# genomematt/xenomapper

Hardware: AMD Instinct MI355X
Metric: read-pairs/sec classified (higher is better)
Workload: dtype int32; 1 GPU; configs[1]: 50000000 PE 2x150 pairs/GPU, AS/XS, liberal, HBM-resident; pairs_per_gpu=50000000, step=xm_classify_compact_dev: classify+count, scan, scatter (3 launches)

## Files before the change

xenomapper_amd/csrc/xm_kernels.hip:

```cpp
#include <hip/hip_runtime.h>
#include <stdint.h>
#include <stdlib.h>

#include "xm_kernels.h"

namespace xm {

template <typename T>
__device__ __forceinline__ uint32_t mapping_state(T a1, T x1, T a2, T x2, T m)
{
    const bool low1 = a1 <= m;
    const bool low2 = a2 <= m;
    const bool prim = (a1 > m) && (low2 || a1 > a2);
    const bool sec  = (a2 > m) && (low1 || a2 > a1);
    const bool spec1 = (x1 == T(0)) || (a1 > x1);
    const bool spec2 = (x2 == T(0)) || (a2 > x2);
    uint32_t s = 6u;
    s = sec ? (spec2 ? 1u : 3u) : s;
    s = (a1 == a2) ? 4u : s;
    s = prim ? (spec1 ? 0u : 2u) : s;
    s = (low1 && low2) ? 5u : s;
    return s;
}

template <>
__device__ __forceinline__ uint32_t mapping_state<int32_t>(int32_t a1, int32_t x1, int32_t a2, int32_t x2, int32_t m)
{
    const bool low1 = a1 <= m, low2 = a2 <= m;
    const bool gt = a1 > a2, lt = a2 > a1;
    const bool spec1 = (x1 == 0) || (a1 > x1);
    const bool spec2 = (x2 == 0) || (a2 > x2);
    uint32_t s = spec2 ? 1u : 3u;
    s = (gt || lt) ? s : 4u;
    s = (!low1 && (low2 || gt)) ? (spec1 ? 0u : 2u) : s;
    s = (low1 && low2) ? 5u : s;
    return s;
}

__device__ __forceinline__ uint32_t bin_of_code(int mode, uint32_t c)
{
    const uint32_t f = (c >> 3) & 7u, r = c & 7u;
    const uint32_t lo = f < r ? f : r;
    const uint32_t hi = f < r ? r : f;
    uint32_t b;
    if (mode == XM_MODE_SE) {
        b = r > 6u ? 6u : r;
    } else if (mode == XM_MODE_PE_LIBERAL) {
        b = lo;
    } else {
        b = (hi == 5u) ? 5u
          : ((hi == 4u) || (((f ^ r) & 1u) != 0u)) ? 4u
          : lo;
    }
    if (mode != XM_MODE_SE) b = (hi > 5u) ? 6u : b;
    return (c == XM_NO_UNIT) ? 7u : b;
}

template <typename T> struct Vec4;
typedef int32_t v4i32 __attribute__((ext_vector_type(4)));
typedef int32_t v4i32_a4 __attribute__((ext_vector_type(4), aligned(4)));
typedef uint32_t v8u32_a4 __attribute__((ext_vector_type(8), aligned(4)));
typedef double  v4f64 __attribute__((ext_vector_type(4)));
template <> struct Vec4<int32_t> { typedef v4i32 type; };
template <> struct Vec4<double>  { typedef v4f64 type; };

template <typename T> __device__ __forceinline__ T absent_value();
template <> __device__ __forceinline__ int32_t absent_value<int32_t>() { return INT32_MIN; }
template <> __device__ __forceinline__ double  absent_value<double>()  { return -__builtin_huge_val(); }

template <typename T, bool NT, bool FULL = false>
__device__ __forceinline__ void load4(const T *__restrict__ col, uint64_t r0, uint64_t n, T out[4])
{
    typedef typename Vec4<T>::type V;
    if (FULL || r0 + 4 <= n) {
        const V *p = reinterpret_cast<const V *>(col + r0);
        const V v = NT ? __builtin_nontemporal_load(p) : *p;
        out[0] = v.x; out[1] = v.y; out[2] = v.z; out[3] = v.w;
    } else {
#pragma unroll
        for (int j = 0; j < 4; ++j) out[j] = (r0 + j < n) ? col[r0 + j] : absent_value<T>();
    }
}

template <typename T, bool NT>
__device__ __forceinline__ void load4_wg(const T *__restrict__ wg, uint32_t byte_off, T out[4])
{
    typedef typename Vec4<T>::type V;
    const V *p = reinterpret_cast<const V *>(reinterpret_cast<const char *>(wg) + byte_off);
    const V v = NT ? __builtin_nontemporal_load(p) : *p;
    out[0] = v.x; out[1] = v.y; out[2] = v.z; out[3] = v.w;
}

__device__ __forceinline__ uint32_t wave_scan_incl(uint32_t v)
{
    v += (uint32_t)__builtin_amdgcn_update_dpp(0, (int)v, 0x111, 0xf, 0xf, false);
    v += (uint32_t)__builtin_amdgcn_update_dpp(0, (int)v, 0x112, 0xf, 0xf, false);
    v += (uint32_t)__builtin_amdgcn_update_dpp(0, (int)v, 0x114, 0xf, 0xf, false);
    v += (uint32_t)__builtin_amdgcn_update_dpp(0, (int)v, 0x118, 0xf, 0xf, false);
    v += (uint32_t)__builtin_amdgcn_update_dpp(0, (int)v, 0x142, 0xa, 0xf, false);
    v += (uint32_t)__builtin_amdgcn_update_dpp(0, (int)v, 0x143, 0xc, 0xf, false);
    return v;
}

__device__ __forceinline__ uint32_t lane_value(uint32_t v, int lane)
{
    return (uint32_t)__builtin_amdgcn_readlane((int)v, lane);
}

#ifdef XM_LOCKSTEP_HOST
__device__ __forceinline__ void lds_settle(int line = __builtin_LINE()) { ls::settle(line); }
#else
__device__ __forceinline__ void lds_settle()
{
    asm volatile("s_waitcnt lgkmcnt(0)" ::: "memory");
}
#endif

#ifdef XM_LOCKSTEP_HOST
#define XM_LAUNCH(kernel, grid, block, st, ...) do { (void)(st); ls::launch(grid, block, [&] { kernel(__VA_ARGS__); }); } while (0)
#else
#define XM_LAUNCH(kernel, grid, block, st, ...) kernel<<<grid, block, 0, st>>>(__VA_ARGS__)
#endif

#if defined(XM_LOCKSTEP_HOST) && defined(LS_SUBSETS)
#define XM_IF_LANES(cond) if (ls::Subset xm_lanes_{static_cast<bool>(cond), __builtin_LINE()}; xm_lanes_.taken)
#else
#define XM_IF_LANES(cond) if (cond)
#endif

#define XM_HREP 8
#define XM_COUNT_LDS_WORDS (64 * XM_HREP + 16)

struct CountSink {
    uint32_t *gran_counts;
    uint32_t *part_tot;
    unsigned long long *counts_rep;
    uint8_t *bins4;
    uint32_t gran_stride;
    int mode;
    uint32_t blk0;
};

__device__ __forceinline__ void count_flush(uint32_t *lds, uint32_t granule, const CountSink &sink)
{
    const uint32_t lane = threadIdx.x & 63u;
    uint32_t *misc = lds + 64 * XM_HREP;
    const uint4 h0 = *reinterpret_cast<const uint4 *>(lds + lane * XM_HREP);
    const uint4 h1 = *reinterpret_cast<const uint4 *>(lds + lane * XM_HREP + 4);
    const uint32_t s = h0.x + h0.y + h0.z + h0.w + h1.x + h1.y + h1.z + h1.w;
    if (s != 0u) {
        atomicAdd(&sink.counts_rep[(granule % XM_COUNT_REPLICAS) * 64u + lane], (unsigned long long)s);
        atomicAdd(&misc[8u + bin_of_code(sink.mode, lane)], s);
    }
    lds_settle();
    if (lane < 8u) {
        const uint32_t v = misc[8u + lane];
        sink.gran_counts[(uint64_t)lane * sink.gran_stride + granule] = v;
        if (v != 0u) atomicAdd(&sink.part_tot[((granule & (XM_PART_REPLICAS - 1u)) * 8u + lane) * XM_PART_STRIDE + granule / XM_PART_GRAN], v);
    }
}

template <int BLOCK>
__device__ __forceinline__ void count_units(const uint32_t c[4], uint32_t *lds, const CountSink &sink)
{
    const uint32_t lane = threadIdx.x & 63u;
    const uint32_t rep = lane & (XM_HREP - 1u);
#pragma unroll
    for (int j = 0; j < 4; ++j) {
        const bool unit = c[j] != XM_NO_UNIT;
        if (__ballot(unit) == 0ull) continue;
        if (unit) atomicAdd(&lds[(c[j] & 63u) * XM_HREP + rep], 1u);
    }
    lds_settle();
    uint32_t arrived = 0;
    if (lane == 0u) arrived = atomicAdd(&lds[64 * XM_HREP], 1u);
    arrived = (uint32_t)__builtin_amdgcn_readfirstlane((int)arrived);
    if (arrived != (uint32_t)(BLOCK / 64 - 1)) return;
    lds_settle();
    count_flush(lds, blockIdx.x + sink.blk0, sink);
}

template <int MODE, bool HAS6>
__device__ __forceinline__ uint32_t unit_bin(uint32_t c)
{
    if (MODE == XM_MODE_SE) return c == XM_NO_UNIT ? 7u : (c & 7u);
    const uint32_t f = (c >> 3) & 7u, r = c & 7u;
    const uint32_t lo = f < r ? f : r, hi = f < r ? r : f;
    uint32_t b = lo;
    if (MODE == XM_MODE_PE_CONSERVATIVE) {
        b = (((f ^ r) & 1u) != 0u || hi == 4u) ? 4u : b;
        b = (hi == 5u) ? 5u : b;
    }
    if (HAS6) b = (hi > 5u) ? 6u : b;
    return c == XM_NO_UNIT ? 7u : b;
}

template <int MODE, bool HAS6>
__device__ __forceinline__ uint32_t unit_bin_of(uint32_t f, uint32_t r, bool unit)
{
    uint32_t b;
    if (MODE == XM_MODE_SE) {
        b = r;
    } else {
        const uint32_t lo = f < r ? f : r, hi = f < r ? r : f;
        b = lo;
        if (MODE == XM_MODE_PE_CONSERVATIVE) {
            b = (((f ^ r) & 1u) != 0u || hi == 4u) ? 4u : b;
            b = (hi == 5u) ? 5u : b;
        }
        if (HAS6) b = (hi > 5u) ? 6u : b;
    }
    return unit ? b : 7u;
}

template <typename T, bool PAIRED, int BLOCK, bool FULL, bool COUNTS, int BINMODE>
__device__ __forceinline__ void classify_finish(const T a1[4], const T x1[4], const T a2[4], const T x2[4], T m,
                                                uint32_t mb, uint32_t halo, uint32_t *last_state,
                                                uint8_t *__restrict__ code, uint64_t r0, uint64_t n,
                                                uint32_t *count_lds, const CountSink &sink)
{
    const uint32_t lane = threadIdx.x & 63u;
    const uint32_t wave = threadIdx.x >> 6;
    uint32_t s[4];
#pragma unroll
    for (int j = 0; j < 4; ++j) s[j] = mapping_state<T>(a1[j], x1[j], a2[j], x2[j], m);

    uint32_t c[4], fwd[4] = {0, 0, 0, 0};
    if (PAIRED) {
        uint32_t prev = (uint32_t)__builtin_amdgcn_update_dpp(0, (int)s[3], 0x138, 0xf, 0xf, false);
        if (lane == 63) last_state[wave] = s[3];
        __syncthreads();
        if (lane == 0) prev = (wave == 0) ? halo : last_state[wave - 1];
        c[0] = (mb & 1u) ? ((prev << 3) | s[0]) : XM_NO_UNIT;
        c[1] = (mb & 2u) ? ((s[0] << 3) | s[1]) : XM_NO_UNIT;
        c[2] = (mb & 4u) ? ((s[1] << 3) | s[2]) : XM_NO_UNIT;
        c[3] = (mb & 8u) ? ((s[2] << 3) | s[3]) : XM_NO_UNIT;
        fwd[0] = prev; fwd[1] = s[0]; fwd[2] = s[1]; fwd[3] = s[2];
    } else {
        if (COUNTS) __syncthreads();
#pragma unroll
        for (int j = 0; j < 4; ++j) c[j] = ((mb >> j) & 1u) ? s[j] : XM_NO_UNIT;
    }

    if (FULL || r0 + 4 <= n) {
        if (code != nullptr) *reinterpret_cast<uint32_t *>(code + r0) = c[0] | (c[1] << 8) | (c[2] << 16) | (c[3] << 24);
    } else {
#pragma unroll
        for (int j = 0; j < 4; ++j)
            if (code != nullptr && r0 + j < n) code[r0 + j] = (uint8_t)c[j];
    }
    if (BINMODE >= 0) {
        uint32_t nib = 0;
#pragma unroll
        for (int j = 0; j < 4; ++j) nib |= unit_bin_of<BINMODE, sizeof(T) == 8>(fwd[j], s[j], ((mb >> j) & 1u) != 0u) << (4 * j);
        reinterpret_cast<uint16_t *>(sink.bins4)[r0 >> 2] = (uint16_t)nib;
    }
    if (COUNTS) count_units<BLOCK>(c, count_lds, sink);
}

template <typename T, bool PAIRED, bool NT, int BLOCK, bool FULL>
__device__ __forceinline__ void classify_load(const T *__restrict__ as1, const T *__restrict__ xs1,
                                              const T *__restrict__ as2, const T *__restrict__ xs2,
                                              const uint8_t *__restrict__ unit_bits8, T m, uint64_t n, uint64_t wg,
                                              T a1[4], T x1[4], T a2[4], T x2[4], uint32_t &mb, uint32_t &halo)
{
    const uint64_t g = wg * BLOCK + threadIdx.x;
    const uint64_t r0 = g * 4;
    mb = 0;
    halo = 0;
    if (FULL) {
        const uint32_t wave = (uint32_t)__builtin_amdgcn_readfirstlane((int)(threadIdx.x >> 6));
        const uint32_t lane = threadIdx.x & 63u;
        const v8u32_a4 mw = *reinterpret_cast<const v8u32_a4 *>(unit_bits8 + wg * (BLOCK / 2) + wave * 32u);
        load4<T, NT, true>(as1, r0, n, a1);
        load4<T, NT, true>(xs1, r0, n, x1);
        load4<T, NT, true>(as2, r0, n, a2);
        load4<T, NT, true>(xs2, r0, n, x2);
        uint32_t d = mw[0];
#pragma unroll
        for (uint32_t k = 1; k < 8u; ++k) d = ((lane >> 3) == k) ? mw[k] : d;
        mb = (d >> ((lane & 7u) * 4u)) & 0xFu;
        if (PAIRED && wave == 0u) {
            if (wg == 0) {
                if (lane == 0u) mb &= ~1u;
            } else if (mw[0] & 1u) {
                const uint64_t h = wg * (BLOCK * 4) - 1;
                halo = mapping_state<T>(as1[h], xs1[h], as2[h], xs2[h], m);
            }
        }
    } else {
        if (r0 < n) mb = (uint32_t)(unit_bits8[g >> 1] >> ((g & 1u) * 4u)) & 0xFu;
        load4<T, NT, false>(as1, r0, n, a1);
        load4<T, NT, false>(xs1, r0, n, x1);
        load4<T, NT, false>(as2, r0, n, a2);
        load4<T, NT, false>(xs2, r0, n, x2);
        if (r0 + 4 > n) mb &= (r0 < n) ? ((1u << (uint32_t)(n - r0)) - 1u) : 0u;
        if (PAIRED && threadIdx.x == 0) {
            if (r0 == 0) {
                mb &= ~1u;
            } else if (mb & 1u) {
                const uint64_t h = r0 - 1;
                halo = mapping_state<T>(as1[h], xs1[h], as2[h], xs2[h], m);
            }
        }
    }
}

template <typename T, bool PAIRED, bool NT, int BLOCK, bool FULL, bool COUNTS, int BINMODE>
__device__ __forceinline__ void classify_body(const T *__restrict__ as1, const T *__restrict__ xs1,
                                              const T *__restrict__ as2, const T *__restrict__ xs2,
                                              const uint8_t *__restrict__ unit_bits8, T m,
                                              uint8_t *__restrict__ code, uint64_t n, uint32_t *last_state,
                                              uint32_t *count_lds, const CountSink &sink)
{
    const uint64_t wg = (uint64_t)blockIdx.x + sink.blk0;
    const uint64_t r0 = (wg * BLOCK + threadIdx.x) * 4;
    T a1[4], x1[4], a2[4], x2[4];
    uint32_t mb, halo;
    classify_load<T, PAIRED, NT, BLOCK, FULL>(as1, xs1, as2, xs2, unit_bits8, m, n, wg, a1, x1, a2, x2, mb, halo);
    classify_finish<T, PAIRED, BLOCK, FULL, COUNTS, BINMODE>(a1, x1, a2, x2, m, mb, halo, last_state, code, r0, n, count_lds, sink);
}

template <int BLOCK>
__device__ __forceinline__ void count_lds_clear(uint32_t *count_lds)
{
    for (uint32_t k = threadIdx.x; k < (uint32_t)XM_COUNT_LDS_WORDS; k += BLOCK) count_lds[k] = 0;
}

template <typename T, bool PAIRED, bool NT, int BLOCK, bool COUNTS, int BINMODE>
__global__ void __launch_bounds__(BLOCK)
classify_kernel(const T *__restrict__ as1, const T *__restrict__ xs1,
                const T *__restrict__ as2, const T *__restrict__ xs2,
                const uint8_t *__restrict__ unit_bits8, T m,
                uint8_t *__restrict__ code, uint64_t n, CountSink sink)
{
    __shared__ uint32_t last_state[BLOCK / 64];
    __shared__ __attribute__((aligned(16))) uint32_t count_lds[COUNTS ? XM_COUNT_LDS_WORDS : 4];
    if (COUNTS) count_lds_clear<BLOCK>(count_lds);
    if (((uint64_t)blockIdx.x + sink.blk0 + 1) * (BLOCK * 4) <= n)
        classify_body<T, PAIRED, NT, BLOCK, true, COUNTS, BINMODE>(as1, xs1, as2, xs2, unit_bits8, m, code, n, last_state, count_lds, sink);
    else
        classify_body<T, PAIRED, NT, BLOCK, false, COUNTS, BINMODE>(as1, xs1, as2, xs2, unit_bits8, m, code, n, last_state, count_lds, sink);
}


__device__ __attribute__((noinline)) uint4 load_codes16_tail(const uint8_t *__restrict__ code, uint64_t base, uint64_t n)
{
    uint32_t w[4];
    for (int k = 0; k < 4; ++k) {
        uint32_t acc = 0;
        for (int j = 0; j < 4; ++j) {
            const uint64_t i = base + 4 * k + j;
            const uint32_t c = (i < n) ? (uint32_t)code[i] : XM_NO_UNIT;
            acc |= c << (8 * j);
        }
        w[k] = acc;
    }
    return make_uint4(w[0], w[1], w[2], w[3]);
}

__device__ __forceinline__ void load_codes16(const uint8_t *__restrict__ code, uint64_t base, uint64_t n,
                                             uint32_t w[4])
{
    uint4 v;
    if (base + 16 <= n) v = *reinterpret_cast<const uint4 *>(code + base);
    else v = load_codes16_tail(code, base, n);
    w[0] = v.x; w[1] = v.y; w[2] = v.z; w[3] = v.w;
}

__device__ __attribute__((noinline)) uint32_t load_codes4_tail(const uint8_t *__restrict__ code, uint64_t base, uint64_t n)
{
    uint32_t acc = 0;
    for (int j = 0; j < 4; ++j) {
        const uint64_t i = base + j;
        const uint32_t c = (i < n) ? (uint32_t)code[i] : XM_NO_UNIT;
        acc |= c << (8 * j);
    }
    return acc;
}

__global__ void __launch_bounds__(XM_BLOCK)
hist_kernel(const uint8_t *__restrict__ code, uint64_t n, uint32_t n_gran, CountSink sink)
{
    __shared__ __attribute__((aligned(16))) uint32_t lds_all[XM_BLOCK / 64][XM_COUNT_LDS_WORDS];
    const uint32_t lane = threadIdx.x & 63u, wave = threadIdx.x >> 6;
    uint32_t *lds = lds_all[wave];
    const uint32_t g = blockIdx.x * (XM_BLOCK / 64) + wave;
    if (g >= n_gran) return;
    for (uint32_t k = lane; k < (uint32_t)XM_COUNT_LDS_WORDS; k += 64u) lds[k] = 0;

    constexpr int TILES = XM_GRAN / 1024;
    const uint64_t rec0 = (uint64_t)g * XM_GRAN;
    uint32_t w[TILES][4];
#pragma unroll
    for (int k = 0; k < TILES; ++k) load_codes16(code, rec0 + (uint64_t)k * 1024u + lane * 16u, n, w[k]);
    lds_settle();

    const uint32_t rep = lane & (XM_HREP - 1u);
    uint32_t common = w[0][0] & 0xFFu;
    if (common == XM_NO_UNIT) common = (w[0][0] >> 8) & 0xFFu;
    common = (uint32_t)__builtin_amdgcn_readfirstlane((int)common);
    uint32_t n_common = 0;
#pragma unroll
    for (int k = 0; k < TILES; ++k) {
#pragma unroll
        for (int j = 0; j < 16; ++j) {
            const uint32_t c = (w[k][j >> 2] >> (8 * (j & 3))) & 0xFFu;
            const bool unit = c != XM_NO_UNIT;
            if (__ballot(unit) == 0ull) continue;
            const bool same = unit && c == common;
            n_common += same ? 1u : 0u;
            if (unit && !same) atomicAdd(&lds[(c & 63u) * XM_HREP + rep], 1u);
        }
    }
    if (n_common) atomicAdd(&lds[(common & 63u) * XM_HREP + rep], n_common);
    lds_settle();
    count_flush(lds, g, sink);
}

#define XM_SCAN_THREADS 1024
__device__ __forceinline__ unsigned long long block_sum_1024(unsigned long long v, unsigned long long *wsum)
{
    v += __shfl_xor(v, 1, 64);  v += __shfl_xor(v, 2, 64);  v += __shfl_xor(v, 4, 64);
    v += __shfl_xor(v, 8, 64);  v += __shfl_xor(v, 16, 64); v += __shfl_xor(v, 32, 64);
    if ((threadIdx.x & 63u) == 0u) wsum[threadIdx.x >> 6] = v;
    __syncthreads();
    unsigned long long total = 0;
#pragma unroll
    for (int w = 0; w < XM_SCAN_THREADS / 64; ++w) total += wsum[w];
    return total;
}

__global__ void __launch_bounds__(XM_SCAN_THREADS)
scan_kernel(const uint32_t *__restrict__ gran_counts, uint32_t n_gran, uint32_t gran_stride,
            const uint32_t *__restrict__ part_tot, uint32_t *__restrict__ gran_off,
            unsigned long long *__restrict__ bin_totals,
            unsigned long long *__restrict__ counts_rep, unsigned long long *__restrict__ counts, uint32_t part0, uint32_t n_parts)
{
    __shared__ unsigned long long wsum[XM_SCAN_THREADS / 64];
    __shared__ uint32_t wtot[XM_SCAN_THREADS / 64];
    const uint32_t p = blockIdx.x + part0, b = blockIdx.y;
    const uint32_t t = threadIdx.x, lane = t & 63u, wave = t >> 6;
    if (p + 1u == n_parts && t < 64u) {
        const uint32_t slot = b * 8u + (t >> 3), part = t & 7u;
        unsigned long long acc = 0;
        for (uint32_t r = part; r < XM_COUNT_REPLICAS; r += 8u) {
            acc += counts_rep[r * 64u + slot];
            counts_rep[r * 64u + slot] = 0;
        }
        acc += __shfl_xor(acc, 1, 64);
        acc += __shfl_xor(acc, 2, 64);
        acc += __shfl_xor(acc, 4, 64);
        if (part == 0) counts[slot] = acc;
    }
    const uint32_t g = p * XM_PART_GRAN + t;
    const uint32_t x = (g < n_gran) ? gran_counts[(uint64_t)b * gran_stride + g] : 0u;
    unsigned long long part_sum = 0;
    for (uint32_t e = t; e < p * XM_PART_REPLICAS; e += XM_SCAN_THREADS) {
        const uint32_t r = e / p, q = e - r * p;
        part_sum += part_tot[(r * 8u + b) * XM_PART_STRIDE + q];
    }
    const unsigned long long carry = block_sum_1024(part_sum, wsum);

    const uint32_t incl = wave_scan_incl(x);
    if (lane == 63u) wtot[wave] = incl;
    __syncthreads();
    uint32_t before_wave = 0, part_total = 0;
    for (uint32_t w = 0; w < XM_SCAN_THREADS / 64; ++w) {
        const uint32_t v = wtot[w];
        before_wave += (w < wave) ? v : 0u;
        part_total += v;
    }
    if (g < n_gran) gran_off[(uint64_t)b * gran_stride + g] = (uint32_t)carry + before_wave + incl - x;
    if (p + 1u == n_parts && t == 0u) bin_totals[b] = carry + part_total;
}

#ifndef XM_SCATTER_GUARD
#define XM_SCATTER_GUARD 1
#endif
__device__ __forceinline__ uint32_t mbcnt64(uint64_t mask, uint32_t add)
{
    return __builtin_amdgcn_mbcnt_hi((uint32_t)(mask >> 32), __builtin_amdgcn_mbcnt_lo((uint32_t)mask, add));
}

template <bool WIDE>
__device__ __forceinline__ void store_index(uint32_t *__restrict__ idx_out, uint32_t pos, uint32_t rec)
{
    if (WIDE) idx_out[pos] = rec;
    else *reinterpret_cast<uint32_t *>(reinterpret_cast<char *>(idx_out) + (pos << 2)) = rec;
}
// ... 957 lines not shown
__device__ __forceinline__ uint32_t cigp_trailer(const uint32_t *__restrict__ ops, uint32_t n_ops, uint32_t end)
{
    return (end > 0u && end <= n_ops) ? (ops[end - 1u] >> 4) : 0u;
}

__device__ __forceinline__ v4i32 cigp_slow(const uint32_t *__restrict__ ops, uint32_t n_ops, uint32_t tb, uint32_t te,
                                                     uint32_t cw, v4i32 nmv, uint32_t *range_flag)
{
    const uint32_t lane = threadIdx.x & 63u;
    if (te > n_ops) te = n_ops;
    if (tb > te) tb = te;
    const uint32_t c0 = cw & 255u, c1 = (cw >> 8) & 255u, c2 = (cw >> 16) & 255u, c3 = cw >> 24;
    uint32_t b0, b1, b2, b3, e0, e1, e2, e3;
    if (__ballot(c0 == 255u || c1 == 255u || c2 == 255u || c3 == 255u) == 0ull) {
        const uint32_t lsum = c0 + c1 + c2 + c3;
        b0 = tb + wave_scan_incl(lsum) - lsum;
        e0 = b1 = b0 + c0; e1 = b2 = b1 + c1; e2 = b3 = b2 + c2; e3 = b3 + c3;
    } else {
        b0 = b1 = b2 = b3 = e0 = e1 = e2 = e3 = tb;
        uint32_t end = te;
        for (int L = 63; L >= 0; --L) {
            const uint32_t w = lane_value(cw, L);
#pragma unroll
            for (int j = 3; j >= 0; --j) {
                uint32_t k = (w >> (8 * j)) & 255u, e = end;
                if (k == 255u) { k = cigp_trailer(ops, n_ops, end); e = end > tb ? end - 1u : tb; }
                const uint32_t b = (e - tb >= k) ? e - k : tb;
                if (lane == (uint32_t)L) {
                    if (j == 0) { b0 = b; e0 = e; } else if (j == 1) { b1 = b; e1 = e; }
                    else if (j == 2) { b2 = b; e2 = e; } else { b3 = b; e3 = e; }
                }
                end = b;
            }
        }
    }
    v4i32 r;
    r.x = cigp_score_range(ops, n_ops, nmv.x, b0, e0, range_flag);
    r.y = cigp_score_range(ops, n_ops, nmv.y, b1, e1, range_flag);
    r.z = cigp_score_range(ops, n_ops, nmv.z, b2, e2, range_flag);
    r.w = cigp_score_range(ops, n_ops, nmv.w, b3, e3, range_flag);
    return r;
}

__device__ __attribute__((noinline)) int32_t cigp_score_before(const int32_t *__restrict__ nm, const uint8_t *__restrict__ cnt,
                                                               const uint32_t *__restrict__ ops, uint32_t n_ops, uint64_t h,
                                                               uint32_t end, uint32_t *range_flag)
{
    if (end > n_ops) end = n_ops;
    uint32_t k = cnt[h], e = end;
    if (k == 255u) { k = cigp_trailer(ops, n_ops, end); e = end > 0u ? end - 1u : 0u; }
    return cigp_score_range(ops, n_ops, nm[h], e >= k ? e - k : 0u, e, range_flag);
}

template <bool FULL>
__device__ __forceinline__ uint32_t cigp_counts4(const uint8_t *__restrict__ cnt, uint64_t r0, uint64_t n)
{
    if (FULL || r0 + 4 <= n) return __builtin_nontemporal_load(reinterpret_cast<const uint32_t *>(cnt + r0));
    uint32_t w = 0;
#pragma unroll
    for (int j = 0; j < 4; ++j)
        if (r0 + j < n) w |= (uint32_t)cnt[r0 + j] << (8 * j);
    return w;
}

template <bool PAIRED, int BLOCK, bool FULL, bool COUNTS, int BINMODE>
__device__ __forceinline__ void classify_cigp_body(const CigCols s1, const CigCols s2, const uint8_t *__restrict__ unit_bits8,
                                                   int32_t m, uint8_t *__restrict__ code, uint64_t n, uint32_t n_tiles,
                                                   uint32_t *__restrict__ range_flag, uint32_t *last_state, uint32_t *cig_T,
                                                   uint32_t *count_lds, const CountSink &sink)
{
    const uint32_t wave = (uint32_t)__builtin_amdgcn_readfirstlane((int)(threadIdx.x >> 6));
    const uint32_t t = blockIdx.x * (BLOCK / 64) + wave;
    const uint64_t g = (uint64_t)blockIdx.x * BLOCK + threadIdx.x;
    const uint64_t r0 = g * 4;
    const bool have_tile = FULL || t < n_tiles;
    const uint32_t lane = threadIdx.x & 63u;

    int32_t a1[4], x1[4], a2[4], x2[4], nmv1[4], nmv2[4];
    uint32_t cw1, cw2, mb = 0;
    const uint64_t wg0 = (uint64_t)blockIdx.x * (BLOCK * 4);
    const uint32_t t16 = threadIdx.x * 16u, t4 = threadIdx.x * 4u;
    if (FULL) {
        load4_wg<int32_t, true>(s1.nm + wg0, t16, nmv1);
        load4_wg<int32_t, true>(s2.nm + wg0, t16, nmv2);
        cw1 = __builtin_nontemporal_load(reinterpret_cast<const uint32_t *>(s1.cnt + wg0 + t4));
        cw2 = __builtin_nontemporal_load(reinterpret_cast<const uint32_t *>(s2.cnt + wg0 + t4));
    } else {
        load4<int32_t, true, false>(s1.nm, r0, n, nmv1);
        load4<int32_t, true, false>(s2.nm, r0, n, nmv2);
        cw1 = cigp_counts4<false>(s1.cnt, r0, n);
        cw2 = cigp_counts4<false>(s2.cnt, r0, n);
    }
    TileOps o1, o2;
    o1.tb = o1.te = o2.tb = o2.te = 0u;
    const uint32_t n_ops1 = s1.tile[n_tiles], n_ops2 = s2.tile[n_tiles];
    if (have_tile) { o1.tb = s1.tile[t]; o1.te = s1.tile[t + 1u]; o2.tb = s2.tile[t]; o2.te = s2.tile[t + 1u]; }
    o1.fast = FULL && o1.te >= o1.tb && o1.te - o1.tb < (uint32_t)XM_CIG_WAVE_OPS && (uint64_t)o1.te + 8u <= n_ops1;
    o2.fast = FULL && o2.te >= o2.tb && o2.te - o2.tb < (uint32_t)XM_CIG_WAVE_OPS && (uint64_t)o2.te + 8u <= n_ops2;
#ifndef XM_CIGP_BRIEF
#define XM_CIGP_BRIEF 1
#endif
    o1.brief = XM_CIGP_BRIEF && o1.fast && o1.te - o1.tb < 256u;
    o2.brief = XM_CIGP_BRIEF && o2.fast && o2.te - o2.tb < 256u;
    if (o1.brief) cigp_load4(s1.ops, o1.tb, o1.te - o1.tb, 4u * lane, o1.v);
    else if (o1.fast) cigp_load8(s1.ops, o1.tb, o1.te - o1.tb, 8u * lane, o1.v);
    if (o2.brief) cigp_load4(s2.ops, o2.tb, o2.te - o2.tb, 4u * lane, o2.v);
    else if (o2.fast) cigp_load8(s2.ops, o2.tb, o2.te - o2.tb, 8u * lane, o2.v);

    bool bad = false;
    if (!(o1.fast && cigp_fast(s1.ops, o1, cw1, nmv1, cig_T, a1, bad))) {
        v4i32 q; q.x = nmv1[0]; q.y = nmv1[1]; q.z = nmv1[2]; q.w = nmv1[3];
        q = cigp_slow(s1.ops, n_ops1, o1.tb, o1.te, cw1, q, range_flag);
        a1[0] = q.x; a1[1] = q.y; a1[2] = q.z; a1[3] = q.w;
    }
    if (FULL) {
        load4_wg<int32_t, true>(s1.xs + wg0, t16, x1);
        load4_wg<int32_t, true>(s2.xs + wg0, t16, x2);
        mb = (uint32_t)((unit_bits8 + (wg0 >> 3))[threadIdx.x >> 1] >> ((threadIdx.x & 1u) * 4u)) & 0xFu;
    } else {
        load4<int32_t, true, false>(s1.xs, r0, n, x1);
        load4<int32_t, true, false>(s2.xs, r0, n, x2);
        if (r0 < n) mb = (uint32_t)(unit_bits8[g >> 1] >> ((g & 1u) * 4u)) & 0xFu;
        if (r0 + 4 > n) mb &= (r0 < n) ? ((1u << (uint32_t)(n - r0)) - 1u) : 0u;
    }
    if (!(o2.fast && cigp_fast(s2.ops, o2, cw2, nmv2, cig_T, a2, bad))) {
        v4i32 q; q.x = nmv2[0]; q.y = nmv2[1]; q.z = nmv2[2]; q.w = nmv2[3];
        q = cigp_slow(s2.ops, n_ops2, o2.tb, o2.te, cw2, q, range_flag);
        a2[0] = q.x; a2[1] = q.y; a2[2] = q.z; a2[3] = q.w;
    }
    if (__ballot(bad) != 0ull && (threadIdx.x & 63u) == 0u && range_flag) atomicOr(range_flag, 1u);

    uint32_t halo = 0;
    if (PAIRED && threadIdx.x == 0) {
        if (r0 == 0) {
            mb &= ~1u;
        } else if (mb & 1u) {
            const uint64_t h = r0 - 1;
            halo = mapping_state<int32_t>(cigp_score_before(s1.nm, s1.cnt, s1.ops, n_ops1, h, o1.tb, range_flag), s1.xs[h],
                                          cigp_score_before(s2.nm, s2.cnt, s2.ops, n_ops2, h, o2.tb, range_flag), s2.xs[h], m);
        }
    }
    classify_finish<int32_t, PAIRED, BLOCK, FULL, COUNTS, BINMODE>(a1, x1, a2, x2, m, mb, halo, last_state, code, r0, n,
                                                                   count_lds, sink);
}

template <bool PAIRED, int BLOCK, bool COUNTS, int BINMODE>
__global__ void __launch_bounds__(BLOCK)
classify_cigp_kernel(const CigCols s1, const CigCols s2, const uint8_t *__restrict__ unit_bits8, int32_t m,
                     uint8_t *__restrict__ code, uint64_t n, uint32_t n_tiles, uint32_t *__restrict__ range_flag, CountSink sink)
{
    static_assert(!COUNTS || BLOCK * 4 == XM_GRAN, "the counting workgroup is one granule");
    __shared__ uint32_t last_state[BLOCK / 64];
    __shared__ __attribute__((aligned(16))) uint32_t cig_table[BLOCK / 64][XM_CIG_WAVE_OPS + 8];
    __shared__ __attribute__((aligned(16))) uint32_t count_lds[COUNTS ? XM_COUNT_LDS_WORDS : 4];
    uint32_t *cig_T = cig_table[threadIdx.x >> 6];
    if (COUNTS) count_lds_clear<BLOCK>(count_lds);
    if (((uint64_t)blockIdx.x + 1) * (BLOCK * 4) <= n)
        classify_cigp_body<PAIRED, BLOCK, true, COUNTS, BINMODE>(s1, s2, unit_bits8, m, code, n, n_tiles, range_flag, last_state,
                                                                 cig_T, count_lds, sink);
    else
        classify_cigp_body<PAIRED, BLOCK, false, COUNTS, BINMODE>(s1, s2, unit_bits8, m, code, n, n_tiles, range_flag, last_state,
                                                                  cig_T, count_lds, sink);
}

#define XM_CORR_T 256
#define XM_CORR_M 2048
__global__ void __launch_bounds__(XM_CORR_T)
mate_correlate_kernel(const double *__restrict__ track, uint64_t n, const double *__restrict__ density, uint32_t m,
                      double *__restrict__ out)
{
#pragma clang fp contract(off)
    __shared__ double tile[XM_CORR_T + XM_CORR_M];
    const uint32_t t = threadIdx.x;
    const uint64_t i0 = (uint64_t)blockIdx.x * XM_CORR_T, i = i0 + t;
    const uint64_t left = (i < n) ? n - i : 0;
    double acc = 0.0;
    for (uint32_t j0 = 0; j0 < m; j0 += XM_CORR_M) {
        const uint32_t mm = (m - j0 < XM_CORR_M) ? m - j0 : XM_CORR_M;
        __syncthreads();
        for (uint32_t k = t; k < XM_CORR_T + mm; k += XM_CORR_T) {
            const uint64_t p = i0 + j0 + k;
            tile[k] = (p < n) ? track[p] : 0.0;
        }
        __syncthreads();
        const uint32_t lim = (left > j0) ? (uint32_t)((left - j0 < mm) ? left - j0 : mm) : 0u;
        if (__ballot(lim != mm) == 0ull) {
            for (uint32_t j = 0; j < mm; ++j) {
                const double prod = tile[t + j] * density[j0 + j];
                acc = acc + prod;
            }
        } else {
            for (uint32_t j = 0; j < mm; ++j) {
                const double prod = tile[t + j] * density[j0 + j];
                const double s = acc + prod;
                acc = (j < lim) ? s : acc;
            }
        }
    }
    if (i < n) out[i] = (track[i] == 1.0) ? 1.0 : acc;
}

__global__ void __launch_bounds__(XM_CLASSIFY_BLOCK)
stream_probe_kernel(const v4i32 *__restrict__ c0, const v4i32 *__restrict__ c1, const v4i32 *__restrict__ c2,
                    const v4i32 *__restrict__ c3, uint16_t *__restrict__ out, uint64_t n_groups)
{
    const uint64_t g = (uint64_t)blockIdx.x * XM_CLASSIFY_BLOCK + threadIdx.x;
    if (g >= n_groups) return;
    const v4i32 a = __builtin_nontemporal_load(c0 + g), b = __builtin_nontemporal_load(c1 + g);
    const v4i32 c = __builtin_nontemporal_load(c2 + g), d = __builtin_nontemporal_load(c3 + g);
    const v4i32 x = a ^ b ^ c ^ d;
    out[g] = (uint16_t)(x.x ^ x.y ^ x.z ^ x.w);
}

void launch_stream_probe(hipStream_t st, uint64_t n, const int32_t *c0, const int32_t *c1, const int32_t *c2, const int32_t *c3,
                         uint8_t *out)
{
    const uint64_t n_groups = n / 4;
    const uint32_t grid = (uint32_t)((n_groups + XM_CLASSIFY_BLOCK - 1) / XM_CLASSIFY_BLOCK);
    if (grid == 0) return;
    XM_LAUNCH(stream_probe_kernel, grid, XM_CLASSIFY_BLOCK, st, reinterpret_cast<const v4i32 *>(c0), reinterpret_cast<const v4i32 *>(c1),
                                                            reinterpret_cast<const v4i32 *>(c2), reinterpret_cast<const v4i32 *>(c3),
                                                            reinterpret_cast<uint16_t *>(out), n_groups);
}

static_assert(XM_CLASSIFY_BLOCK * 4 == XM_GRAN, "the counting classify workgroup is one granule");

GranPlan plan_granules(uint64_t n)
{
    GranPlan p;
    uint64_t g = (n + XM_GRAN - 1) / XM_GRAN;
    if (g == 0) g = 1;
    p.n_gran = (uint32_t)g;
    p.gran_stride = (p.n_gran + 63u) & ~63u;
    return p;
}

static CountSink make_sink(const CountPlan *cp, int mode)
{
    CountSink s;
    s.gran_counts = cp ? cp->gran_counts : nullptr;
    s.part_tot = cp ? cp->part_tot : nullptr;
    s.counts_rep = cp ? reinterpret_cast<unsigned long long *>(cp->counts_rep) : nullptr;
    s.bins4 = cp ? cp->bins4 : nullptr;
    s.gran_stride = cp ? cp->plan.gran_stride : 0u;
    s.mode = mode;
    s.blk0 = cp ? cp->gran0 : 0u;
    return s;
}

template <typename T>
void launch_classify(hipStream_t st, int mode, uint64_t n, const T *as1, const T *xs1, const T *as2, const T *xs2,
                     const uint64_t *unit_bits, T m, uint8_t *code, const CountPlan *cp)
{
    const uint64_t per_block = (uint64_t)XM_CLASSIFY_BLOCK * 4;
    static_assert(XM_CLASSIFY_BLOCK * 4 == XM_GRAN, "a counting workgroup is a granule: CountPlan's chunk is in both");
    const uint32_t all = (uint32_t)((n + per_block - 1) / per_block);
    const uint32_t grid = (cp && cp->gran1) ? cp->gran1 - cp->gran0 : all;
    const uint8_t *bits8 = reinterpret_cast<const uint8_t *>(unit_bits);
    const CountSink sink = make_sink(cp, mode);
    const bool paired = mode != XM_MODE_SE;
#define XM_LAUNCH_CLS(P, C, B) XM_LAUNCH((classify_kernel<T, P, XM_CLASSIFY_NT, XM_CLASSIFY_BLOCK, C, B>), grid, XM_CLASSIFY_BLOCK, st, as1, xs1, as2, xs2, bits8, m, code, n, sink)
    if (cp && cp->bins4) {
        if (mode == XM_MODE_SE) XM_LAUNCH_CLS(false, true, XM_MODE_SE);
        else if (mode == XM_MODE_PE_LIBERAL) XM_LAUNCH_CLS(true, true, XM_MODE_PE_LIBERAL);
        else XM_LAUNCH_CLS(true, true, XM_MODE_PE_CONSERVATIVE);
    }
    else if (cp) { if (paired) XM_LAUNCH_CLS(true, true, -1); else XM_LAUNCH_CLS(false, true, -1); }
    else         { if (paired) XM_LAUNCH_CLS(true, false, -1); else XM_LAUNCH_CLS(false, false, -1); }
#undef XM_LAUNCH_CLS
}

template void launch_classify<int32_t>(hipStream_t, int, uint64_t, const int32_t *, const int32_t *, const int32_t *, const int32_t *,
                                       const uint64_t *, int32_t, uint8_t *, const CountPlan *);
template void launch_classify<double>(hipStream_t, int, uint64_t, const double *, const double *, const double *, const double *,
                                      const uint64_t *, double, uint8_t *, const CountPlan *);

template <typename T>
void launch_classify_runs(hipStream_t st, int mode, uint64_t n, const T *as1, const T *xs1, const T *as2, const T *xs2,
                          const uint64_t *unit_bits, T m, const RunsOut &ro)
{
    const uint64_t per_block = (uint64_t)XM_CLASSIFY_BLOCK * 4;
    const uint32_t grid = (uint32_t)((n + per_block - 1) / per_block);
    const uint8_t *bits8 = reinterpret_cast<const uint8_t *>(unit_bits);
    RunsSink rs;
    rs.runs16 = ro.runs16;
    rs.gran_counts16 = ro.gran_counts16;
    rs.counts_rep = reinterpret_cast<unsigned long long *>(ro.counts_rep);
#define XM_LAUNCH_RUNS(P, B) XM_LAUNCH((classify_runs_kernel<T, P, XM_CLASSIFY_NT, XM_CLASSIFY_BLOCK, B>), grid, XM_CLASSIFY_BLOCK, st, as1, xs1, as2, xs2, bits8, m, n, rs)
    if (mode == XM_MODE_SE) XM_LAUNCH_RUNS(false, XM_MODE_SE);
    else if (mode == XM_MODE_PE_LIBERAL) XM_LAUNCH_RUNS(true, XM_MODE_PE_LIBERAL);
    else XM_LAUNCH_RUNS(true, XM_MODE_PE_CONSERVATIVE);
#undef XM_LAUNCH_RUNS
}

template void launch_classify_runs<int32_t>(hipStream_t, int, uint64_t, const int32_t *, const int32_t *, const int32_t *,
                                            const int32_t *, const uint64_t *, int32_t, const RunsOut &);
template void launch_classify_runs<double>(hipStream_t, int, uint64_t, const double *, const double *, const double *,
                                           const double *, const uint64_t *, double, const RunsOut &);

void launch_runs_finish(hipStream_t st, int mode, uint64_t *counts_rep, uint64_t *counts, uint64_t *n_out)
{
    XM_LAUNCH(runs_finish_kernel, 1, 256, st, reinterpret_cast<unsigned long long *>(counts_rep),
                                          reinterpret_cast<unsigned long long *>(counts),
                                          reinterpret_cast<unsigned long long *>(n_out), mode);
}

void launch_classify_cigar(hipStream_t st, int mode, uint64_t n,
// ... 102 lines not shown
```

Before: 153.2 billion read-pairs/s.

## Restructure classify counting with per-wave histograms, majority-value ballots and early flush

Reworks the counting path of the classify kernel. Each wave gets its own histogram column, and a wave-uniform majority code is tallied with a ballot plus popcount so only outliers issue LDS atomics. When every wave's paired units avoid the cross-wave halo slots, the block takes an early path. There it computes per-wave bin counts with ballots and flushes granule counts through DPP reductions after one barrier, skipping the arrival-counter flush. This aims to cut LDS atomic contention and the serialized last-wave flush, at the cost of more complex control flow and an extra barrier and LDS flag array.

Result: no change. 151.7 billion read-pairs/s (-1.0%).

```diff
diff --git a/xenomapper_amd/csrc/xm_kernels.hip b/xenomapper_amd/csrc/xm_kernels.hip
--- a/xenomapper_amd/csrc/xm_kernels.hip
+++ b/xenomapper_amd/csrc/xm_kernels.hip
@@ -130,6 +130,9 @@
 
 #define XM_HREP 8
 #define XM_COUNT_LDS_WORDS (64 * XM_HREP + 16)
+#define XM_K1_WBINS_AT XM_COUNT_LDS_WORDS
+#define XM_K1_FLAGS_AT (XM_K1_WBINS_AT + 64)
+#define XM_K1_LDS_WORDS (XM_K1_FLAGS_AT + 8)
 
 struct CountSink {
     uint32_t *gran_counts;
@@ -161,19 +164,80 @@
 }
 
 template <int BLOCK>
-__device__ __forceinline__ void count_units(const uint32_t c[4], uint32_t *lds, const CountSink &sink)
+__device__ __forceinline__ void count_lds_clear(uint32_t *lds)
+{
+    static_assert(BLOCK / 64 == XM_HREP, "one histogram column per wave");
+    lds[(threadIdx.x & 63u) * XM_HREP + (threadIdx.x >> 6)] = 0;
+    if (threadIdx.x < 16u) lds[64 * XM_HREP + threadIdx.x] = 0;
+}
+
+template <int SLOTS>
+__device__ __forceinline__ void count_wave(const uint32_t c[4], uint32_t *col)
+{
+    constexpr int J0 = (SLOTS & 1) ? 0 : 1, J1 = (SLOTS & 1) ? 1 : 3;
+    uint32_t common = c[J0] != XM_NO_UNIT ? c[J0] : c[J1];
+    common = (uint32_t)__builtin_amdgcn_readfirstlane((int)common);
+    uint32_t n_common = 0;
+#pragma unroll
+    for (int j = 0; j < 4; ++j) {
+        if (!((SLOTS >> j) & 1)) continue;
+        const bool unit = c[j] != XM_NO_UNIT;
+        const bool same = unit && c[j] == common;
+        n_common += (uint32_t)__builtin_popcountll(__ballot(same));
+        if (unit && !same) atomicAdd(&col[(c[j] & 63u) * XM_HREP], 1u);
+    }
+    if ((threadIdx.x & 63u) == 0u && n_common != 0u) atomicAdd(&col[(common & 63u) * XM_HREP], n_common);
+}
+
+template <int SLOTS, int NB>
+__device__ __forceinline__ uint32_t wave_bin_counts(const uint32_t bin[4])
 {
     const uint32_t lane = threadIdx.x & 63u;
-    const uint32_t rep = lane & (XM_HREP - 1u);
-#pragma unroll
-    for (int j = 0; j < 4; ++j) {
-        const bool unit = c[j] != XM_NO_UNIT;
-        if (__ballot(unit) == 0ull) continue;
-        if (unit) atomicAdd(&lds[(c[j] & 63u) * XM_HREP + rep], 1u);
-    }
+    uint32_t wc = 0;
+#pragma unroll
+    for (int b = 0; b < NB; ++b) {
+        uint32_t total = 0;
+#pragma unroll
+        for (int j = 0; j < 4; ++j)
+            if ((SLOTS >> j) & 1) total += (uint32_t)__builtin_popcountll(__ballot(bin[j] == (uint32_t)b));
+        wc = (lane == (uint32_t)b) ? total : wc;
+    }
+    return wc;
+}
+
+__device__ __forceinline__ uint32_t sum8_dpp(uint32_t v)
+{
+    v += (uint32_t)__builtin_amdgcn_update_dpp(0, (int)v, 0x111, 0xf, 0xf, false);
+    v += (uint32_t)__builtin_amdgcn_update_dpp(0, (int)v, 0x112, 0xf, 0xf, false);
+    v += (uint32_t)__builtin_amdgcn_update_dpp(0, (int)v, 0x114, 0xf, 0xf, false);
+    return v;
+}
+
+__device__ __forceinline__ void count_flush_early(const uint32_t *lds, uint32_t wave, uint32_t granule, const CountSink &sink)
+{
+    const uint32_t lane = threadIdx.x & 63u;
+    uint32_t v = lds[64u * wave + lane];
+    uint32_t wb = 0;
+    if (wave == 0u) wb = lds[XM_K1_WBINS_AT + (lane & 7u) * 8u + (lane >> 3)];
+    v = sum8_dpp(v);
+    if ((lane & 7u) == 7u && v != 0u)
+        atomicAdd(&sink.counts_rep[(granule % XM_COUNT_REPLICAS) * 64u + 8u * wave + (lane >> 3)], (unsigned long long)v);
+    if (wave == 0u) {
+        wb = sum8_dpp(wb);
+        if ((lane & 7u) == 7u) {
+            const uint32_t b = lane >> 3;
+            sink.gran_counts[(uint64_t)b * sink.gran_stride + granule] = wb;
+            if (wb != 0u) atomicAdd(&sink.part_tot[((granule & (XM_PART_REPLICAS - 1u)) * 8u + b) * XM_PART_STRIDE + granule / XM_PART_GRAN], wb);
+        }
+    }
+}
+
+template <int BLOCK>
+__device__ __forceinline__ void count_arrive(uint32_t *lds, const CountSink &sink)
+{
     lds_settle();
     uint32_t arrived = 0;
-    if (lane == 0u) arrived = atomicAdd(&lds[64 * XM_HREP], 1u);
+    if ((threadIdx.x & 63u) == 0u) arrived = atomicAdd(&lds[64 * XM_HREP], 1u);
     arrived = (uint32_t)__builtin_amdgcn_readfirstlane((int)arrived);
     if (arrived != (uint32_t)(BLOCK / 64 - 1)) return;
     lds_settle();
@@ -213,6 +277,88 @@
     return unit ? b : 7u;
 }
 
+template <typename T, bool FULL, int BINMODE>
+__device__ __forceinline__ void classify_store(const uint32_t c[4], const uint32_t fwd[4], const uint32_t s[4], uint32_t mb,
+                                               uint8_t *__restrict__ code, uint64_t r0, uint64_t n, const CountSink &sink)
+{
+    if (FULL || r0 + 4 <= n) {
+        if (code != nullptr) *reinterpret_cast<uint32_t *>(code + r0) = c[0] | (c[1] << 8) | (c[2] << 16) | (c[3] << 24);
+    } else {
+#pragma unroll
+        for (int j = 0; j < 4; ++j)
+            if (code != nullptr && r0 + j < n) code[r0 + j] = (uint8_t)c[j];
+    }
+    if (BINMODE >= 0) {
+        uint32_t nib = 0;
+#pragma unroll
+        for (int j = 0; j < 4; ++j) nib |= unit_bin_of<BINMODE, sizeof(T) == 8>(fwd[j], s[j], ((mb >> j) & 1u) != 0u) << (4 * j);
+        reinterpret_cast<uint16_t *>(sink.bins4)[r0 >> 2] = (uint16_t)nib;
+    }
+}
+
+template <typename T, bool PAIRED, int BLOCK, bool FULL, int BINMODE>
+__device__ __forceinline__ void classify_finish_counting(const uint32_t s[4], uint32_t mb, uint32_t halo, uint32_t *last_state,
+                                                         uint8_t *__restrict__ code, uint64_t r0, uint64_t n,
+                                                         uint32_t *count_lds, const CountSink &sink)
+{
+    constexpr bool HAS6 = sizeof(T) == 8;
+    constexpr int NB = (HAS6 || BINMODE < 0) ? 7 : 6;
+    constexpr int EARLY_SLOTS = PAIRED ? 0xA : 0xF;
+    const uint32_t lane = threadIdx.x & 63u;
+    const uint32_t wave = (uint32_t)__builtin_amdgcn_readfirstlane((int)(threadIdx.x >> 6));
+    uint32_t *col = count_lds + wave;
+    const bool early = FULL && (!PAIRED || __ballot((mb & 5u) != 0u) == 0ull);
+
+    uint32_t c[4], fwd[4] = {0, 0, 0, 0};
+    uint32_t prev = 0;
+    if (PAIRED) {
+        prev = (uint32_t)__builtin_amdgcn_update_dpp(0, (int)s[3], 0x138, 0xf, 0xf, false);
+        if (lane == 63) last_state[wave] = s[3];
+    }
+    if (early) {
+        if (PAIRED) {
+            c[0] = XM_NO_UNIT;
+            c[1] = (mb & 2u) ? ((s[0] << 3) | s[1]) : XM_NO_UNIT;
+            c[2] = XM_NO_UNIT;
+            c[3] = (mb & 8u) ? ((s[2] << 3) | s[3]) : XM_NO_UNIT;
+            fwd[1] = s[0]; fwd[3] = s[2];
+        } else {
+#pragma unroll
+            for (int j = 0; j < 4; ++j) c[j] = ((mb >> j) & 1u) ? s[j] : XM_NO_UNIT;
+        }
+        classify_store<T, FULL, BINMODE>(c, fwd, s, mb, code, r0, n, sink);
+        count_wave<EARLY_SLOTS>(c, col);
+        uint32_t bin[4];
+#pragma unroll
+        for (int j = 0; j < 4; ++j)
+            bin[j] = BINMODE >= 0 ? unit_bin_of<BINMODE, HAS6>(fwd[j], s[j], ((mb >> j) & 1u) != 0u) : bin_of_code(sink.mode, c[j]);
+        const uint32_t wc = wave_bin_counts<EARLY_SLOTS, NB>(bin);
+        if (lane < 8u) count_lds[XM_K1_WBINS_AT + wave * 8u + lane] = wc;
+    }
+    if (FULL && lane == 0u) count_lds[XM_K1_FLAGS_AT + wave] = early ? 1u : 0u;
+    __syncthreads();
+    if (FULL && __ballot(count_lds[XM_K1_FLAGS_AT + (lane & 7u)] == 0u) == 0ull) {
+        count_flush_early(count_lds, wave, blockIdx.x + sink.blk0, sink);
+        return;
+    }
+    if (!early) {
+        if (PAIRED) {
+            if (lane == 0) prev = (wave == 0) ? halo : last_state[wave - 1];
+            c[0] = (mb & 1u) ? ((prev << 3) | s[0]) : XM_NO_UNIT;
+            c[1] = (mb & 2u) ? ((s[0] << 3) | s[1]) : XM_NO_UNIT;
+            c[2] = (mb & 4u) ? ((s[1] << 3) | s[2]) : XM_NO_UNIT;
+            c[3] = (mb & 8u) ? ((s[2] << 3) | s[3]) : XM_NO_UNIT;
+            fwd[0] = prev; fwd[1] = s[0]; fwd[2] = s[1]; fwd[3] = s[2];
+        } else {
+#pragma unroll
+            for (int j = 0; j < 4; ++j) c[j] = ((mb >> j) & 1u) ? s[j] : XM_NO_UNIT;
+        }
+        classify_store<T, FULL, BINMODE>(c, fwd, s, mb, code, r0, n, sink);
+        count_wave<0xF>(c, col);
+    }
+    count_arrive<BLOCK>(count_lds, sink);
+}
+
 template <typename T, bool PAIRED, int BLOCK, bool FULL, bool COUNTS, int BINMODE>
 __device__ __forceinline__ void classify_finish(const T a1[4], const T x1[4], const T a2[4], const T x2[4], T m,
                                                 uint32_t mb, uint32_t halo, uint32_t *last_state,
@@ -224,6 +370,10 @@
     uint32_t s[4];
 #pragma unroll
     for (int j = 0; j < 4; ++j) s[j] = mapping_state<T>(a1[j], x1[j], a2[j], x2[j], m);
+    if (COUNTS) {
+        classify_finish_counting<T, PAIRED, BLOCK, FULL, BINMODE>(s, mb, halo, last_state, code, r0, n, count_lds, sink);
+        return;
+    }
 
     uint32_t c[4], fwd[4] = {0, 0, 0, 0};
     if (PAIRED) {
@@ -237,11 +387,11 @@
         c[3] = (mb & 8u) ? ((s[2] << 3) | s[3]) : XM_NO_UNIT;
         fwd[0] = prev; fwd[1] = s[0]; fwd[2] = s[1]; fwd[3] = s[2];
     } else {
-        if (COUNTS) __syncthreads();
 #pragma unroll
         for (int j = 0; j < 4; ++j) c[j] = ((mb >> j) & 1u) ? s[j] : XM_NO_UNIT;
     }
 
+    static_assert(COUNTS || BINMODE < 0, "the compact stream comes from the counting kernels only");
     if (FULL || r0 + 4 <= n) {
         if (code != nullptr) *reinterpret_cast<uint32_t *>(code + r0) = c[0] | (c[1] << 8) | (c[2] << 16) | (c[3] << 24);
     } else {
@@ -249,13 +399,6 @@
         for (int j = 0; j < 4; ++j)
             if (code != nullptr && r0 + j < n) code[r0 + j] = (uint8_t)c[j];
     }
-    if (BINMODE >= 0) {
-        uint32_t nib = 0;
-#pragma unroll
-        for (int j = 0; j < 4; ++j) nib |= unit_bin_of<BINMODE, sizeof(T) == 8>(fwd[j], s[j], ((mb >> j) & 1u) != 0u) << (4 * j);
-        reinterpret_cast<uint16_t *>(sink.bins4)[r0 >> 2] = (uint16_t)nib;
-    }
-    if (COUNTS) count_units<BLOCK>(c, count_lds, sink);
 }
 
 template <typename T, bool PAIRED, bool NT, int BLOCK, bool FULL>
@@ -321,12 +464,6 @@
     classify_finish<T, PAIRED, BLOCK, FULL, COUNTS, BINMODE>(a1, x1, a2, x2, m, mb, halo, last_state, code, r0, n, count_lds, sink);
 }
 
-template <int BLOCK>
-__device__ __forceinline__ void count_lds_clear(uint32_t *count_lds)
-{
-    for (uint32_t k = threadIdx.x; k < (uint32_t)XM_COUNT_LDS_WORDS; k += BLOCK) count_lds[k] = 0;
-}
-
 template <typename T, bool PAIRED, bool NT, int BLOCK, bool COUNTS, int BINMODE>
 __global__ void __launch_bounds__(BLOCK)
 classify_kernel(const T *__restrict__ as1, const T *__restrict__ xs1,
@@ -335,7 +472,7 @@
                 uint8_t *__restrict__ code, uint64_t n, CountSink sink)
 {
     __shared__ uint32_t last_state[BLOCK / 64];
-    __shared__ __attribute__((aligned(16))) uint32_t count_lds[COUNTS ? XM_COUNT_LDS_WORDS : 4];
+    __shared__ __attribute__((aligned(16))) uint32_t count_lds[COUNTS ? XM_K1_LDS_WORDS : 4];
     if (COUNTS) count_lds_clear<BLOCK>(count_lds);
     if (((uint64_t)blockIdx.x + sink.blk0 + 1) * (BLOCK * 4) <= n)
         classify_body<T, PAIRED, NT, BLOCK, true, COUNTS, BINMODE>(as1, xs1, as2, xs2, unit_bits8, m, code, n, last_state, count_lds, sink);
@@ -1599,7 +1736,7 @@
     static_assert(!COUNTS || BLOCK * 4 == XM_GRAN, "the counting workgroup is one granule");
     __shared__ uint32_t last_state[BLOCK / 64];
     __shared__ __attribute__((aligned(16))) uint32_t cig_table[BLOCK / 64][XM_CIG_WAVE_OPS + 8];
-    __shared__ __attribute__((aligned(16))) uint32_t count_lds[COUNTS ? XM_COUNT_LDS_WORDS : 4];
+    __shared__ __attribute__((aligned(16))) uint32_t count_lds[COUNTS ? XM_K1_LDS_WORDS : 4];
     uint32_t *cig_T = cig_table[threadIdx.x >> 6];
     if (COUNTS) count_lds_clear<BLOCK>(count_lds);
     if (((uint64_t)blockIdx.x + 1) * (BLOCK * 4) <= n)
```
